# Jingliang-Duan/DSAC-v2

Measured on AMD Instinct MI355X. Metric: DSAC-T gradient steps/sec, batch=256 Humanoid (obs376/act17), higher is better.
Workload: dtype f32

## Files before the change

### dsac-v2_amd/csrc/dsact_api.hip

```cpp
#include <hip/hip_runtime.h>
#include <hip/hip_ext.h>
#include <dlfcn.h>
#include <chrono>
#include <stdarg.h>
#include <stdio.h>
#include <math.h>
#include <stdlib.h>
#include <string.h>

#include <algorithm>
#include <atomic>
#include <string>
#include <vector>

#include "../../include/dsact.h"
#include "dsact_kernels.h"
#include "dsact_chain.h"
#include "dsact_fat.h"
#include "dsact_act.h"
#include "dsact_act_batch.h"
#include "dsact_host_act.h"
#include "dsact_conv.h"

#define DSACT_KERNEL(group, ...) extern template __global__ void __VA_ARGS__;
// ... 2899 lines not shown
  if (cfg->conv_type != DSACT_CONV_NONE) {
    static const int k1[] = {8, 4, 3}, c1[] = {32, 64, 64}, s1[] = {4, 2, 1};
    static const int k2[] = {4, 3, 3, 3, 3, 3}, c2[] = {8, 16, 32, 64, 128, 256}, s2[] = {2, 2, 2, 2, 1, 1};
    if (cfg->conv_type != DSACT_CONV_TYPE_1 && cfg->conv_type != DSACT_CONV_TYPE_2) return fail(h, DSACT_E_INVALID, "conv_type must be 0, 1 (type_1) or 2 (type_2)");
    const bool t1 = cfg->conv_type == DSACT_CONV_TYPE_1;
    const int* ks = t1 ? k1 : k2; const int* cs = t1 ? c1 : c2; const int* ss = t1 ? s1 : s2;
    h->n_conv = t1 ? 3 : 6;
    if (cfg->img_c < 1 || cfg->img_h < 1 || cfg->img_w < 1 || (long long)cfg->img_c * cfg->img_h * cfg->img_w != cfg->obs_dim)
      return fail(h, DSACT_E_INVALID, "obs_dim must equal img_c*img_h*img_w for CNN nets");
    if (cfg->obs_dim % 4) return fail(h, DSACT_E_INVALID, "img_c*img_h*img_w must be a multiple of 4");
    int C = cfg->img_c, H = cfg->img_h, W = cfg->img_w;
    for (int j = 0; j < h->n_conv; ++j) {
      ConvGeom& g = h->cg[j];
      g.H = H; g.W = W; g.Cin = C; g.KS = ks[j]; g.stride = ss[j]; g.Cout = cs[j];
      g.OH = (H - g.KS) / g.stride + 1; g.OW = (W - g.KS) / g.stride + 1;
      if (H < g.KS || W < g.KS || g.OH < 1 || g.OW < 1) return fail(h, DSACT_E_INVALID, "image %dx%d too small for conv layer %d", cfg->img_h, cfg->img_w, j);
      g.K = g.KS * g.KS * g.Cin; g.KWC = g.KS * g.Cin; g.rowskip = g.W * g.Cin - g.KWC;
      g.inv_kwc = 1.0f / (float)g.KWC;
      if (g.KWC % 4) return fail(h, DSACT_E_INVALID, "kernel_width*channels of conv layer %d must be a multiple of 4 (got %d)", j, g.KWC);
      C = g.Cout; H = g.OH; W = g.OW;
    }
    h->cnn = true;
    h->cP = H * W;
    h->F = C * H * W;
    nblk = 2;
  }
  int pol_hidden[DSACT_MAX_HIDDEN_LAYERS] = {0};
  bool unequal = false;
  h->Lq = cfg->n_hidden;
  h->Lp = cfg->policy_n_hidden > 0 ? cfg->policy_n_hidden : cfg->n_hidden;
  if (h->Lp > DSACT_MAX_HIDDEN_LAYERS) return fail(h, DSACT_E_INVALID, "policy_n_hidden must be 0 (= n_hidden) or 1..%d", DSACT_MAX_HIDDEN_LAYERS);
  if (h->Lp != h->Lq && cfg->conv_type != DSACT_CONV_NONE) return fail(h, DSACT_E_INVALID, "policy_n_hidden: the CNN nets' MLP widths are fixed by conv_type");
  unequal = h->Lp != h->Lq;
  h->L = h->Lp > h->Lq ? h->Lp : h->Lq;
  for (int l = 0; l < h->Lp; ++l) {
    pol_hidden[l] = cfg->policy_hidden[l] > 0 ? cfg->policy_hidden[l] : (l < h->Lq ? cfg->hidden[l] : 0);
    if (pol_hidden[l] < 1 || pol_hidden[l] > kMaxWidth) return fail(h, DSACT_E_INVALID, "policy hidden width of layer %d must be 1..%d", l, kMaxWidth);
    unequal = unequal || l >= h->Lq || pol_hidden[l] != cfg->hidden[l];
  }
  if (unequal && (cfg->conv_type != DSACT_CONV_NONE || cfg->algo != 0))
    return fail(h, DSACT_E_INVALID, "value_hidden_sizes != policy_hidden_sizes is built for DSAC_V2 with MLP nets (tile-stage kernels)");
  const int nblk_pol = cfg->policy_twin ? 2 : nblk;
  h->unequal_widths = unequal || nblk_pol != nblk;
  for (int l = 0; l < h->L; ++l) {
    h->wq[l] = l < h->Lq ? nblk * cfg->hidden[l] : 0; h->wp[l] = l < h->Lp ? nblk_pol * pol_hidden[l] : 0;
    h->w[l] = h->wq[l] > h->wp[l] ? h->wq[l] : h->wp[l];
  }
  for (int l = 0; l < h->L; ++l)
    if (h->w[l] > kMaxWidth) return fail(h, DSACT_E_INVALID, "activation row width %d exceeds %d", h->w[l], kMaxWidth);
  h->ldx = (h->F + h->A + 3) & ~3;
  h->use_w1p = (size_t)4 * nblk * cfg->hidden[0] * h->ldx <= ((size_t)4 << 20);
  build_net(h->qd, h->F + h->A, cfg->hidden, h->Lq, 2, nblk, h->n_conv, h->cg);
  build_net(h->pd, h->F, pol_hidden, h->Lp, 2 * h->A, nblk_pol, h->n_conv, h->cg);
  h->n_q = h->qd.count; h->n_pi = h->pd.count;
  if (cfg->algo != DSACT_ALGO_DSAC_V2 && cfg->algo != DSACT_ALGO_DSAC_V1) return fail(h, DSACT_E_INVALID, "algo must be 0 (DSAC_V2) or 1 (DSAC_V1)");
  h->nq = cfg->algo == DSACT_ALGO_DSAC_V1 ? 1 : 2;
  h->n_online = h->nq * h->n_q + h->n_pi + 1;
  h->n_target = h->nq * h->n_q + h->n_pi;
  h->n_heads_wg = (h->B + 3) / 4;
  h->n_loss_wg = (h->B + 3) / 4;
  h->loss_rows = 4;
  h->auto_std_sums = h->B > 1024;
  if (const char* v = getenv("DSACT_TIMELINE_STAGE")) h->env_timeline_stage = v;
  { int v = 0; if (hipDeviceGetAttribute(&v, hipDeviceAttributeMultiprocessorCount, h->device) == hipSuccess && v > 0) h->n_cu = v; (void)hipGetLastError(); }
  h->env_no_pipe_defer = getenv("DSACT_NO_PIPE_DEFER") != nullptr;
  h->env_no_bqt = getenv("DSACT_NO_BQT_MERGE") != nullptr;
  h->env_no_bqp = getenv("DSACT_NO_BQP_MERGE") != nullptr;
  if (const char* v = getenv("DSACT_PIPE_MAP")) h->env_pipe_map = v;
  h->env_no_dcol_ident = getenv("DSACT_NO_DCOL_IDENT") != nullptr;
  h->env_no_fat_stage = getenv("DSACT_NO_FAT_STAGE") != nullptr;
  h->dw_chunks = (h->B > 448 && h->B % 256 == 0) ? h->B / 256 : 1;
  h->dw_part_stride = (h->n_online + 2 + 63) & ~(size_t)63;
  {
    const int R = 4 * h->cRG;
    bool ok = h->B % R == 0 && h->B % 16 == 0 && (h->B <= 256 || h->B % 256 == 0) &&
              getenv("DSACT_NO_CHAIN") == nullptr && !(h->nq == 1 && getenv("DSACT_NO_CHAIN_V1") != nullptr) &&
              !(h->cnn && (getenv("DSACT_NO_CHAIN_CNN") != nullptr || h->B > 1024));
    ok = ok && h->L <= kChMaxL;
    ok = ok && !h->unequal_widths;
    ok = ok && cfg->value_out_act != OUT_ACT_GELU && cfg->policy_out_act != OUT_ACT_GELU;
    for (int l = 0; l < h->L; ++l) ok = ok && cfg->hidden[l] == cfg->hidden[0];
    const int W0 = cfg->hidden[0];
    ok = ok && (W0 == 64 || W0 == 128 || W0 == 256);
    h->s_obs = roundup((h->F + 3) / 4, kPD);
    h->s_act = roundup((h->A + 3) / 4, kPD);
    h->SoT = roundup((2 * h->A + 3) / 4, kPD);
    ok = ok && (size_t)chain_lds(4 * (h->s_obs + h->s_act), W0, R).total * sizeof(float) <= 150 * 1024;
    h->chain_ok = ok;
    h->twin = ok && h->cnn;
    h->env_twin_seq = getenv("DSACT_TWIN_SEQ") != nullptr;
    if (ok) {
      const int per = (h->B > 1024 && h->B % 1024 == 0) ? 1024 : 256;
      h->dw_chunks = h->B > 1024 ? h->B / per : 1;
    }
    h->cW = W0; h->cNT = W0 / 64; h->n_slices = h->B / R;
    h->rg4_ok = ok && h->B % 16 == 0 &&
                (size_t)chain_lds(4 * (h->s_obs + h->s_act), W0, 16).total * sizeof(float) <= 150 * 1024;
    h->c_obs = (h->F + 15) / 16; h->c_act = (h->A + 15) / 16; h->c_out = (2 * h->A + 15) / 16;
    {
      const char* fm = getenv("DSACT_FAT_MIN");
      const int fat_min = fm ? atoi(fm) : 1024;
      h->fat = ok && !h->cnn && h->nq == 2 && h->B >= fat_min && h->B % 32 == 0 && (W0 == 128 || W0 == 256) &&
               cfg->value_out_act == 0 && cfg->policy_out_act == 0;
      h->fat_bwd = h->fat && h->B >= 4096;
      if (const char* v = getenv("DSACT_FAT_RT")) h->env_fat_rt = atoi(v) == 2 ? 2 : 1;
    }
    h->fwd_merge = ok && !h->cnn && h->B <= 256 && h->B / 4 <= kChainFlagSlices && chain_rg(h, 4) == 1 && getenv("DSACT_NO_FWD_MERGE") == nullptr;
    h->pi_merge = ok && !h->cnn && h->B <= 512 && !h->fat_bwd && getenv("DSACT_NO_PI_MERGE") == nullptr;
  }
  Carver c0;
  carve(h, c0, h->sets[0], SET_WS);
  h->ws_bytes = c0.off + 256;
  HIPCHK(h, hipMalloc(&h->ws, h->ws_bytes));
  HIPCHK(h, hipMemset(h->ws, 0, h->ws_bytes));
  Carver c1;
  c1.base = h->ws;
  carve(h, c1, h->sets[0], SET_WS);
  {
    DevState st0;
    memset(&st0, 0, sizeof(st0));
    st0.b1p_q = st0.b2p_q = st0.b1p_pi = st0.b2p_pi = st0.b1p_alpha = st0.b2p_alpha = 1.0;
    HIPCHK(h, hipMemcpy(h->st, &st0, sizeof(st0), hipMemcpyHostToDevice));
  }
  {
    std::vector<float> ones(h->B, 1.0f);
    HIPCHK(h, hipMemcpy(h->ones, ones.data(), h->B * sizeof(float), hipMemcpyHostToDevice));
  }
  if (h->cnn) {
    for (int j = 0; j < h->n_conv; ++j) {
      const ConvGeom& g = h->cg[j];
      if ((size_t)h->Brows * g.H * g.W * g.Cin > 2147483647ull || (size_t)h->Brows * g.OH * g.OW >= (1u << 24))
        return fail(h, DSACT_E_INVALID, "batch x image too large for the conv index arithmetic (layer %d)", j);
    }
    std::vector<int> iota(h->Brows);
    for (int i = 0; i < h->Brows; ++i) iota[i] = i;
    HIPCHK(h, hipMemcpy(h->idx_iota, iota.data(), iota.size() * sizeof(int), hipMemcpyHostToDevice));
  }
  HIPCHK(h, hipStreamCreateWithFlags(&h->stream, hipStreamNonBlocking));
  h->own_stream = true;
  for (const KernelFamily* f : kernels().all)
    for (int c = 0; c < f->n_cells; ++c)
      if (f->max_lds && f->cells[c]) HIPCHK(h, hipFuncSetAttribute(f->cells[c], hipFuncAttributeMaxDynamicSharedMemorySize, f->max_lds));
  HIPCHK(h, hipHostMalloc((void**)&h->handoff_host, 1024, hipHostMallocMapped));
  memset(h->handoff_host, 0, 1024);
  HIPCHK(h, hipHostGetDevicePointer((void**)&h->handoff_dev, h->handoff_host, 0));
  h->act_out_host = (unsigned long long*)(h->handoff_host + 32); h->act_out_dev = (unsigned long long*)(h->handoff_dev + 32);
  HIPCHK(h, hipMalloc((void**)&h->act_h, (size_t)kActMaxLayers * kMaxWidth * sizeof(unsigned long long)));
  HIPCHK(h, hipMemset(h->act_h, 0, (size_t)kActMaxLayers * kMaxWidth * sizeof(unsigned long long)));
  h->env_no_fast_act = getenv("DSACT_NO_FAST_ACT") != nullptr;
  h->host_act = getenv("DSACT_NO_HOST_ACT") == nullptr;

  if (h->fwd_merge) {
    int per_cu = 0;
    const size_t la = (size_t)chain_lds(4 * (h->s_obs + h->s_act), h->cW, 4 * chain_rg(h, 6)).total * sizeof(float);
    const void* fn = (const void*)kernels().chain_fwd2.find({h->cNT, false});
    if (!fn || hipOccupancyMaxActiveBlocksPerMultiprocessor(&per_cu, fn, 64 * h->cNT, la) != hipSuccess || per_cu < 2) h->fwd_merge = false;
    (void)hipGetLastError();
  }
  for (int i = 0; i < 8; ++i) {
    HIPCHK(h, hipHostMalloc((void**)&h->h_idx[i], (size_t)h->B * sizeof(int), hipHostMallocDefault));
    HIPCHK(h, hipEventCreateWithFlags(&h->h_idx_ev[i], hipEventDisableTiming));
  }
  return DSACT_OK;
}

int dsact_destroy(dsact_handle* h) {
  if (!h) return DSACT_E_INVALID;
  hipSetDevice(h->device);
  if (h->stream) hipStreamSynchronize(h->stream);
// ... 2390 lines not shown
```

### dsac-v2_amd/csrc/dsact_chain.h

```cpp
#pragma once
#include "dsact_kernels.h"

namespace dsact {

#ifndef DSACT_TILE_NAP
#define DSACT_TILE_NAP 24
#endif
constexpr int kChMaxL = 4;
#ifndef DSACT_KPD
#define DSACT_KPD 16
#endif
constexpr int kPD = DSACT_KPD;

#ifdef DSACT_TIMELINE
#define CTL(buf, k) do { if ((buf) && threadIdx.x == 0 && blockIdx.x < 1024) (buf)[blockIdx.x * 16 + (k)] = (long long)__builtin_readcyclecounter(); } while (0)
#define CTLR(buf, k) do { if ((buf) && threadIdx.x == 0 && blockIdx.x < 1024) (buf)[blockIdx.x * 16 + (k)] = (long long)__builtin_amdgcn_s_memrealtime(); } while (0)
#define CTLV(buf, k, v) do { if ((buf) && threadIdx.x == 0 && blockIdx.x < 1024) (buf)[blockIdx.x * 16 + (k)] = (long long)(v); } while (0)
#else
#define CTL(buf, k) do {} while (0)
#define CTLR(buf, k) do {} while (0)
#define CTLV(buf, k, v) do {} while (0)
#endif


struct WStr { f32x4 b[kPD]; };

__device__ __forceinline__ void stream_prologue(WStr& ws, const float* cur, int s_lo, int lane4) {
#pragma unroll
  for (int u = 0; u < kPD; ++u) ws.b[u] = gload4(cur + (size_t)(s_lo + u) * 256 + lane4);
}

__device__ __forceinline__ const float* uniform_ptr(const float* p) {
  const unsigned long long v = (unsigned long long)p;
  const unsigned lo = __builtin_amdgcn_readfirstlane((unsigned)v), hi = __builtin_amdgcn_readfirstlane((unsigned)(v >> 32));
  return (const float*)(((unsigned long long)hi << 32) | lo);
}
__device__ __forceinline__ const float* sgpr_ptr(const float* p) { p = uniform_ptr(p); asm("" : "+s"(p)); return p; }

template <int RG, bool TAIL = false>
__device__ __forceinline__ void gemm44_seg(WStr& ws, const float* cur, int s_lo, int s_hi, const float* nxt, int nxt_s0,
                                           bool has_nxt, const float* lds, int xs, int ld, int lane4, f32x4 (&acc)[RG][2],
                                           const float* tail = nullptr, int tail_c = 0, int tail_nt = 0) {
  static_assert(!TAIL || kPD >= 8, "the tail takes 8 slots of the stream");
  static_assert(kPD % 4 == 0, "one scalar base per 4 steps");
  constexpr bool SB = RG >= 2;
  f32x4 a0[RG], a1[RG];
#pragma unroll
  for (int g = 0; g < RG; ++g) a0[g] = *(const f32x4*)(lds + xs + 4 * g * ld + 4 * s_lo);
  for (int s0 = s_lo; s0 < s_hi; s0 += kPD) {
    const float* src = s0 + kPD < s_hi ? cur + (size_t)(s0 + kPD) * 256
                                       : (has_nxt ? nxt + (size_t)nxt_s0 * 256 : cur + (size_t)s_lo * 256);
    const bool at_tail = TAIL && tail != nullptr && !has_nxt && !(s0 + kPD < s_hi);
    const float* src8 = at_tail ? tail : src;
    const int tq = at_tail ? (tail_nt > 1 ? tail_c : 0) : 4;
    const float* sb[kPD / 4];
    if (SB) {
#pragma unroll
      for (int k = 0; k < kPD / 4; ++k) sb[k] = sgpr_ptr(TAIL && k < 2 ? src8 + (size_t)(k * tq) * 256 : src + (size_t)k * 1024);
    }
#pragma unroll
    for (int u = 0; u < kPD; ++u) {
      const int s = s0 + u;
#pragma unroll
      for (int g = 0; g < RG; ++g) {
        if (u & 1) a0[g] = *(const f32x4*)(lds + xs + 4 * g * ld + 4 * (s + 1));
        else a1[g] = *(const f32x4*)(lds + xs + 4 * g * ld + 4 * (s + 1));
      }
#pragma unroll
      for (int e = 0; e < 4; ++e) {
#pragma unroll
        for (int g = 0; g < RG; ++g)
          acc[g][e & 1] = __builtin_amdgcn_mfma_f32_4x4x1f32((u & 1) ? a1[g][e] : a0[g][e], ws.b[u][e], acc[g][e & 1], 0, 0, 0);
        if (e == 1) __builtin_amdgcn_sched_barrier(0);
      }
      if (SB) ws.b[u] = gload4(sb[u >> 2] + (size_t)(u & 3) * 256 + lane4);
      else if (TAIL && u < 8) ws.b[u] = gload4(src8 + (size_t)((u >> 2) * tq + (u & 3)) * 256 + lane4);
      else ws.b[u] = gload4(src + (size_t)u * 256 + lane4);
      __builtin_amdgcn_sched_barrier(0);
    }
  }
}

template <int NTO_MAX>
struct NarrowFrags { f32x4 w[NTO_MAX][4]; };

template <int NTO_MAX>
__device__ __forceinline__ void narrow_load(NarrowFrags<NTO_MAX>& f, const float* wf, int C, int nto, int wave, int lane4) {
#pragma unroll
  for (int t = 0; t < NTO_MAX; ++t) {
    if (t < nto) {
#pragma unroll
      for (int c = 0; c < 4; ++c) f.w[t][c] = gload4(wf + ((size_t)t * C + (size_t)wave * 4 + c) * 256 + lane4);
    }
  }
}
template <int NTO_MAX>
__device__ __forceinline__ void narrow_mma(const NarrowFrags<NTO_MAX>& f, int nto, int wave, float* lds, int xs, int red, int lane) {
  f32x4 a[4];
#pragma unroll
  for (int c = 0; c < 4; ++c) a[c] = *(const f32x4*)(lds + xs + 16 * (wave * 4 + c));
#pragma unroll
  for (int t = 0; t < NTO_MAX; ++t) {
    if (t < nto) {
      f32x4 acc = {0.f, 0.f, 0.f, 0.f};
#pragma unroll
      for (int c = 0; c < 4; ++c)
#pragma unroll
        for (int e = 0; e < 4; ++e) acc = __builtin_amdgcn_mfma_f32_16x16x4f32(f.w[t][c][e], a[c][e], acc, 0, 0, 0);
      *(f32x4*)(lds + red + ((wave * NTO_MAX + t) * 64 + lane) * 4) = acc;
    }
  }
}
template <int NTO_MAX, int NW>
__device__ __forceinline__ float narrow_get(const float* lds, int red, int m, int n) {
  const int t = n >> 4, ln = (((n & 15) >> 2) << 4) + m, e = n & 3;
  float s = lds[red + ((0 * NTO_MAX + t) * 64 + ln) * 4 + e];
#pragma unroll
  for (int w = 1; w < NW; ++w) s += lds[red + ((w * NTO_MAX + t) * 64 + ln) * 4 + e];
  return s;
}

template <int TPR>
__device__ __forceinline__ float rowN_sum(float v) {
  v += dpp_mov<0xB1>(v);
  v += dpp_mov<0x4E>(v);
  if (TPR >= 8) v += dpp_mov<0x141>(v);
  if (TPR >= 16) v += dpp_mov<0x140>(v);
  if (TPR >= 32) { float a, b; swap16(v, a, b); v = a + b; }
  if (TPR >= 64) { float a, b; swap32(v, a, b); v = a + b; }
  return v;
}

__device__ __forceinline__ bool chain_decode(int b, int n_units, int n_slices, int& unit, int& slice) {
  const int rep = n_units >= 5 ? 1 : (n_units >= 3 ? 2 : (n_units == 2 ? 4 : 8));
  const int xcd = b & 7, rnd = b >> 3;
  if (xcd >= n_units * rep) return false;
  unit = xcd % n_units;
  slice = rnd * rep + xcd / n_units;
  return slice < n_slices;
}
inline int chain_grid(int n_units, int n_slices) {
  const int rep = n_units >= 5 ? 1 : (n_units >= 3 ? 2 : (n_units == 2 ? 4 : 8));
  return 8 * ((n_slices + rep - 1) / rep);
}
struct XcdMap { int unit[8], base[8], stride[8]; };
inline XcdMap xcd_map_uniform(int n_units) {
  XcdMap m;
  const int rep = n_units >= 5 ? 1 : (n_units >= 3 ? 2 : (n_units == 2 ? 4 : 8));
  for (int x = 0; x < 8; ++x) {
    const bool on = x < n_units * rep;
    m.unit[x] = on ? x % n_units : -1; m.base[x] = on ? x / n_units : 0; m.stride[x] = rep;
  }
  return m;
}
inline XcdMap xcd_map_shares(int n_units, const int* share) {
  XcdMap m;
  int x = 0;
  for (int u = 0; u < n_units; ++u)
    for (int k = 0; k < share[u] && x < 8; ++k, ++x) { m.unit[x] = u; m.base[x] = k; m.stride[x] = share[u]; }
  for (; x < 8; ++x) { m.unit[x] = -1; m.base[x] = 0; m.stride[x] = 1; }
  return m;
// ... 413 lines not shown
      const int a0 = f0 ? __hip_atomic_load(f0, __ATOMIC_RELAXED, __HIP_MEMORY_SCOPE_AGENT) : 1;
      const int a1 = f1 ? __hip_atomic_load(f1, __ATOMIC_RELAXED, __HIP_MEMORY_SCOPE_AGENT) : 1;
      if (a0 && a1) break;
      if (++spins > (1 << 17)) { if (timeout) *timeout = 1; break; }
      __builtin_amdgcn_s_sleep(16);
    }
  }
  __syncthreads();
}

constexpr int kArriveStride = 64;
__device__ __forceinline__ void pack_store4(float* p, const f32x4& v, int agent) {
  if (agent) asm volatile("global_store_dwordx4 %0, %1, off sc1" : : "v"(p), "v"(v) : "memory");
  else nt_store4(p, v);
}
__device__ __forceinline__ void hand_store(float* p, float v, int agent) {
  if (agent) st_agent(p, v); else *p = v;
}
__device__ __forceinline__ void chain_arrive(int* cnt) {
  if (!cnt) return;
  stores_acked_barrier();
  if (threadIdx.x < 8) __hip_atomic_fetch_add(cnt + threadIdx.x * kArriveStride, 1, __ATOMIC_RELAXED, __HIP_MEMORY_SCOPE_AGENT);
}
struct ArriveWait {
  const int* cnt; int need; int* timeout;
  long long* tl = nullptr;
  int quick = 0;
  int kind = 0;
  __device__ __forceinline__ void operator()() const {
    if (threadIdx.x == 0) {
      const int* c = cnt + ((int)blockIdx.x & 7) * kArriveStride;
      int spins = 0;
      while (__hip_atomic_load(c, __ATOMIC_RELAXED, __HIP_MEMORY_SCOPE_AGENT) < need) {
        if (++spins > (1 << 17)) { if (timeout) *timeout = 1; break; }
        if (quick) __builtin_amdgcn_s_sleep(4); else __builtin_amdgcn_s_sleep(DSACT_TILE_NAP);
      }
    }
    asm volatile("s_barrier" ::: "memory");
    CTLR(tl, 13);
  }
  __device__ __forceinline__ void stamp_class(int v) const { CTLV(tl, 11, kind | v); }
};

__device__ __forceinline__ bool fwd_decode(const FwdArgs& a, int b, int& unit, int& slice) {
  const int x = b & 7;
  unit = a.map.unit[x];
  if (unit < 0) return false;
  slice = a.map.base[x] + a.map.stride[x] * (b >> 3);
  return slice < a.u[unit].n_slices;
}
inline int fwd_grid(const FwdArgs& a) {
  int rounds = 0;
  for (int x = 0; x < 8; ++x) {
    if (a.map.unit[x] < 0) continue;
    const int n = a.u[a.map.unit[x]].n_slices - a.map.base[x];
    const int r = n > 0 ? (n + a.map.stride[x] - 1) / a.map.stride[x] : 0;
    rounds = r > rounds ? r : rounds;
  }
  return 8 * rounds;
}

template <int NW, int RG, bool GA = false, typename AT = FwdArgs, typename UT = FwdUnit>
__device__ __forceinline__ void chain_fwd_body(const AT& a, const UT& u, int unit, int slice, float* lds) {
  constexpr int W = 64 * NW, SH = W / 4, R = 4 * RG, NTHR = 64 * NW, TPR = NTHR / R;
  int* const done_flag = (u.done && !(a.debug_withhold && unit == 0 && slice == 0)) ? u.done + slice : nullptr;
  const int tid = threadIdx.x, lane = tid & 63;
  const int wave = __builtin_amdgcn_readfirstlane(tid >> 6);
  const int lane4 = lane * 4;
  const int n = 64 * wave + lane;
  const int row0 = slice * R;
  const int L = a.L, F = a.F, A = a.A;
  const int S0 = a.s_obs + u.s_act;
  const int head = u.head & HEAD_KIND, twin = u.head & (HEAD_TWIN_FIRST | HEAD_TWIN_SECOND);
  const int c_out = ((u.head >> 8) & 0xff) ? ((u.head >> 8) & 0xff) : W / 16;
  const int oact = GA ? head_out_act(u.head) : 0;
  const ChainLds S = chain_lds(4 * (a.s_obs + a.s_act), W, R);
  const int xin = S.off_in, red = S.off_red;
  CTL(a.timeline, 0);
  CTLR(a.timeline, 14);
  const bool do_obs = u.seg != SEG_ACT_FROM_SAVED;
  const bool do_act = u.seg != SEG_OBS_ONLY && u.s_act > 0;
  WStr ws;
  const float* w0 = u.wf[0] + (size_t)wave * (S0 + a.tpad) * 256;
  stream_prologue(ws, w0, do_obs ? 0 : a.s_obs, lane4);
  float bq[kChMaxL];
#pragma unroll
  for (int l = 0; l < kChMaxL; ++l) bq[l] = u.bias[l < L ? l : 0][n];
  const int mr = tid / TPR, jr = tid % TPR;
  constexpr int NQ = (32 + TPR - 1) / TPR;
  float pre_eps[NQ], pre_bmu[NQ], pre_braw[NQ], pre_s[NQ], pre_c[NQ];
#pragma unroll
  for (int q = 0; q < NQ; ++q) { pre_eps[q] = 0.f; pre_bmu[q] = 0.f; pre_braw[q] = 0.f; pre_s[q] = 1.f; pre_c[q] = 0.f; }
  if (head == HEAD_POLICY) {
#pragma unroll
    for (int q = 0; q < NQ; ++q) {
      const int d = jr + q * TPR;
      if (d < A) {
        pre_eps[q] = u.eps[(size_t)(row0 + mr) * A + d];
        pre_bmu[q] = u.bias[L][d]; pre_braw[q] = u.bias[L][A + d];
        pre_s[q] = a.act_scale[d]; pre_c[q] = a.act_center[d];
      }
    }
  } else if (head == HEAD_Q && jr == 0) {
    pre_bmu[0] = u.bias[L][0]; pre_braw[0] = u.bias[L][1];
  }
  const bool pairs_in = (u.late_wait & HW_PAIRS_IN) != 0, pairs_out = (u.late_wait & HW_PAIRS_OUT) != 0;
  const unsigned tag = (pairs_in || pairs_out) ? (unsigned)(*a.tagp) + 1u : 0u;
  const bool head_wait = (u.late_wait & HW_HEAD) != 0;
  const int* const flag0 = (pairs_in || head_wait) ? nullptr : u.wait0;
  const bool waits = flag0 || u.wait1 || pairs_in;
  const bool late = waits && (u.late_wait & HW_LATE) && u.seg != SEG_ACT_FROM_SAVED && u.s_act > 0;
  if ((flag0 || u.wait1) && !late)
    chain_wait(flag0 ? flag0 + row0 / u.wait_rows0 : nullptr, u.wait1 ? u.wait1 + row0 / u.wait_rows1 : nullptr, a.spin_timeout);
  f32x4 zi[RG];
  if (u.seg == SEG_ACT_FROM_SAVED) {
#pragma unroll
    for (int g = 0; g < RG; ++g)
#pragma unroll
      for (int r = 0; r < 4; ++r) zi[g][r] = ld_agent(u.zinit + (size_t)(row0 + 4 * g + r) * W + n);
  }
  auto stage_act = [&]() {
    const int Fp = 4 * a.s_obs;
    if (pairs_in) {
      const unsigned long long* hp = (const unsigned long long*)u.wait0;
      const int per_row = 4 * u.s_act;
      for (int e = tid; e < R * per_row; e += NTHR) {
        const int r = e / per_row, k = e % per_row;
        float v = 0.0f;
        if (k < A) {
          const unsigned long long* src = hp + (size_t)(row0 + r) * 32 + k;
          unsigned long long pv = __hip_atomic_load(src, __ATOMIC_RELAXED, __HIP_MEMORY_SCOPE_AGENT);
          int spins = 0;
          while ((unsigned)(pv >> 32) != tag) {
            if (++spins > (1 << 17)) { if (a.spin_timeout) *a.spin_timeout = 1; break; }
            __builtin_amdgcn_s_sleep(8);
            pv = __hip_atomic_load(src, __ATOMIC_RELAXED, __HIP_MEMORY_SCOPE_AGENT);
          }
          v = __builtin_bit_cast(float, (unsigned)pv);
        }
        lds[xin + r * S.ld_in + Fp + k] = v;
      }
      return;
    }
    const int aq = u.s_act, total = R * aq;
    for (int e = tid; e < total; e += NTHR) {
      const int r = e / aq, k = (e % aq) * 4;
      f32x4 v = {0.f, 0.f, 0.f, 0.f};
      const float* s = u.x + (size_t)(row0 + r) * a.ldx + F + k;
      for (int c = 0; c < 4; ++c) if (k + c < A) v[c] = ld_agent(s + c);
      *(f32x4*)(lds + xin + r * S.ld_in + Fp + k) = v;
    }
  };
  {
    const int Fp = 4 * a.s_obs;
    if (do_obs) {
      const int fq = Fp >> 2, total = R * fq;
      for (int e0 = tid; e0 < total; e0 += 4 * NTHR) {
        f32x4 v[4];
#pragma unroll
        for (int q = 0; q < 4; ++q) {
          const int e = e0 + q * NTHR;
          const int r = e < total ? e / fq : 0, k = e < total ? (e % fq) * 4 : 0;
          const float* s = u.x + (size_t)(row0 + r) * a.ldx + (k + 3 < F ? k : 0);
          v[q] = *(const f32x4u*)s;
        }
#pragma unroll
        for (int q = 0; q < 4; ++q) {
          const int e = e0 + q * NTHR;
          if (e < total) {
            const int r = e / fq, k = (e % fq) * 4;
            f32x4 o = v[q];
            if (k + 3 >= F) {
              const float* s = u.x + (size_t)(row0 + r) * a.ldx;
              for (int c = 0; c < 4; ++c) o[c] = k + c < F ? s[k + c] : 0.0f;
            }
            *(f32x4*)(lds + xin + r * S.ld_in + k) = o;
          }
        }
      }
    }
    if (do_act && !late) stage_act();
  }
  f32x4 acc[RG][2];
#pragma unroll
  for (int g = 0; g < RG; ++g) { acc[g][0] = f32x4{0.f, 0.f, 0.f, 0.f}; acc[g][1] = acc[g][0]; }
  if (u.seg == SEG_ACT_FROM_SAVED) {
#pragma unroll
    for (int g = 0; g < RG; ++g) acc[g][0] = zi[g];
  }
  lds_barrier();
  CTL(a.timeline, 1);
  if (u.x0t) {
    const int K0 = F + (do_act ? A : 0);
    for (int e = tid; e < K0 * RG; e += NTHR) {
      const int k = e / RG, g4 = e % RG;
      const int kk = k < F ? k : 4 * a.s_obs + (k - F);
      f32x4 v;
#pragma unroll
      for (int r = 0; r < 4; ++r) v[r] = lds[xin + (4 * g4 + r) * S.ld_in + kk];
      nt_store4(u.x0t + pk_index(k, row0 + 4 * g4, a.Cb), v);
    }
  }
  const int xs_in = xin + (lane & 3) * S.ld_in;
  const bool more = L > 1;
  const float* w1 = u.wf[more ? 1 : 0] + (size_t)wave * (more ? SH + a.tpad : S0 + a.tpad) * 256;
  if (do_obs) {
    const bool into_act = do_act;
    gemm44_seg<RG>(ws, w0, 0, a.s_obs, into_act ? w0 : w1, into_act ? a.s_obs : 0, into_act || (more && u.seg != SEG_OBS_ONLY),
                   lds, xs_in, S.ld_in, lane4, acc);
    if (u.zsave) {
#pragma unroll
      for (int g = 0; g < RG; ++g) {
        const f32x4 v = acc[g][0] + acc[g][1];
#pragma unroll
        for (int r = 0; r < 4; ++r) st_agent(u.zsave + (size_t)(row0 + 4 * g + r) * W + n, v[r]);
      }
      if (u.zdone) chain_publish(u.zdone + slice);
    }
    CTL(a.timeline, 2);
    if (u.seg == SEG_OBS_ONLY) { CTLR(a.timeline, 15); chain_publish(done_flag); return; }
    if (u.seg == SEG_FULL_SPLIT) {
#pragma unroll
      for (int g = 0; g < RG; ++g) { acc[g][0] = acc[g][0] + acc[g][1]; acc[g][1] = f32x4{0.f, 0.f, 0.f, 0.f}; }
    }
  }
  if (late) {
    if (flag0 || u.wait1)
      chain_wait(flag0 ? flag0 + row0 / u.wait_rows0 : nullptr, u.wait1 ? u.wait1 + row0 / u.wait_rows1 : nullptr, a.spin_timeout);
    stage_act();
    lds_barrier();
  }
  if (do_act) gemm44_seg<RG>(ws, w0, a.s_obs, S0, w1, 0, more, lds, xs_in, S.ld_in, lane4, acc);
  CTL(a.timeline, 3);
  NarrowFrags<4> hf;
  const int nto = head == HEAD_POLICY ? (2 * A + 15) >> 4 : 1;
  for (int l = 0; l < L; ++l) {
    if (l == L - 1 && head != HEAD_NONE) narrow_load<4>(hf, u.wf[L], c_out, nto, wave, lane4);
    const int hn = (l & 1) ? S.off_h1 : S.off_h0;
    const float bl = l == 0 ? bq[0] : l == 1 ? bq[1] : l == 2 ? bq[2] : bq[3];
#pragma unroll
    for (int g = 0; g < RG; ++g) {
      const f32x4 z = acc[g][0] + acc[g][1] + bl;
      f32x4 hv, gd;
      if (GA) act4(u.act, z, hv, gd); else gelu4(z, hv, gd);
#pragma unroll
      for (int r = 0; r < 4; ++r) lds[hn + (4 * g + r) * S.ld_h + n] = hv[r];
      if (u.H[l]) nt_store4(u.H[l] + pk_index(n, row0 + 4 * g, a.Cb), hv);
      if (u.G[l]) nt_store4(u.G[l] + pk_index(n, row0 + 4 * g, a.Cb), gd);
      acc[g][0] = f32x4{0.f, 0.f, 0.f, 0.f}; acc[g][1] = acc[g][0];
    }
    lds_barrier();
    CTL(a.timeline, 4 + 2 * l);
    if (l + 1 < L) {
      const float* wc = u.wf[l + 1] + (size_t)wave * (SH + a.tpad) * 256;
      const bool has_nxt = l + 2 < L;
      const float* wn = u.wf[has_nxt ? l + 2 : l + 1] + (size_t)wave * (SH + a.tpad) * 256;
      gemm44_seg<RG>(ws, wc, 0, SH, wn, 0, has_nxt, lds, hn + (lane & 3) * S.ld_h, S.ld_h, lane4, acc);
      CTL(a.timeline, 5 + 2 * l);
    }
  }
  if (head == HEAD_NONE) { CTLR(a.timeline, 15); chain_publish(done_flag); return; }
  const int hl = ((L - 1) & 1) ? S.off_h1 : S.off_h0;
  narrow_mma<4>(hf, nto, wave, lds, hl + ((lane & 15) & (R - 1)) * S.ld_h + 4 * (lane >> 4), red, lane);
  lds_barrier();
  CTL(a.timeline, 12);
  float* const carry = lds + S.off_carry;
  if (twin == HEAD_TWIN_FIRST) {
    for (int e = tid; e < R * 16 * nto; e += NTHR) {
      const int mm = e / (16 * nto), o = e % (16 * nto);
      const float v = narrow_get<4, NW>(lds, red, mm, o);
      if (u.qout) st_agent(u.qout + (size_t)(row0 + mm) * 64 + o, v);
      else carry[mm * 64 + o] = v;
    }
    CTLR(a.timeline, 15);
    if (u.qout) chain_publish(done_flag);
    return;
  }
  const bool add_carry = twin == HEAD_TWIN_SECOND;
  if (head_wait) {
    chain_wait(u.wait0 + row0 / u.wait_rows0, nullptr, a.spin_timeout);
    for (int e = tid; e < R * 16 * nto; e += NTHR) {
      const int mm = e / (16 * nto), o = e % (16 * nto);
      carry[mm * 64 + o] = ld_agent(u.zinit + (size_t)(row0 + mm) * 64 + o);
    }
    lds_barrier();
  }
  const int m = mr, j = jr;
  const int r = row0 + m;
  if (head == HEAD_Q) {
    if (j == 0) {
      float mean = narrow_get<4, NW>(lds, red, m, 0), raw = narrow_get<4, NW>(lds, red, m, 1);
      if (add_carry) { mean += carry[m * 64]; raw += carry[m * 64 + 1]; }
      mean += pre_bmu[0]; raw += pre_braw[0];
      float sgm = 1.0f;
      if (GA && oact) { mean = out_act_fwd(oact, mean); raw = out_act_fwd(oact, raw); sgm = out_act_grad_y(oact, raw); }
      u.qout[2 * r] = mean; u.qout[2 * r + 1] = raw;
      if (u.qstd) { u.qstd[2 * r] = softplus(raw); u.qstd[2 * r + 1] = softplus_grad(raw) * sgm; }
    }
    CTL(a.timeline, 13);
    CTLR(a.timeline, 15);
    chain_publish(done_flag);
    return;
  }
  float lp = 0.f, s_tanh = 0.f, s_sig = 0.f;
#pragma unroll
  for (int q = 0; q < NQ; ++q) {
    const int d = j + q * TPR;
    if (d >= A) break;
    float mu = narrow_get<4, NW>(lds, red, m, d), raw = narrow_get<4, NW>(lds, red, m, A + d);
    if (add_carry) { mu += carry[m * 64 + d]; raw += carry[m * 64 + A + d]; }
    mu += pre_bmu[q]; raw += pre_braw[q];
    if (GA && oact) { mu = out_act_fwd(oact, mu); if (!(u.head & HEAD_STD_PLAIN)) raw = out_act_fwd(oact, raw); }
    const TanhGaussFwd f = tanh_gauss_fwd(mu, raw, pre_eps[q], pre_s[q], pre_c[q], a.lo_ls, a.hi_ls);
    lp += f.lp;
    st_agent(u.xact + (size_t)r * a.ldx + F + d, f.a);
// ... 359 lines not shown
    } else narrow_load<2>(af, u.w1at, c1at, nta, wave, lane4);
  }
  narrow_mma<2>(af, nta, wave, lds, (cur ? S.off_h1 : S.off_h0) + ((lane & 15) & (R - 1)) * S.ld_h + 4 * (lane >> 4), red, lane);
  lds_barrier();
  const unsigned ptag = (MRG && u.dA_pairs) ? (unsigned)(*a.tagp) + 1u : 0u;
  for (int d = j; d < 16 * nta; d += TPR) {
    const float v = d < a.A ? narrow_get<2, NW>(lds, red, m, d) : 0.0f;
    u.dA[(size_t)r * 32 + d] = v;
    if (MRG && u.dA_pairs)
      __hip_atomic_store(u.dA_pairs + (size_t)r * 32 + d, ((unsigned long long)ptag << 32) | (unsigned long long)__builtin_bit_cast(unsigned, v),
                         __ATOMIC_RELAXED, __HIP_MEMORY_SCOPE_AGENT);
  }
  CTL(a.timeline, 12);
  CTLR(a.timeline, 15);
}

template <int NW, int RG>
__global__ void __launch_bounds__(256) k_chain_bwd_q(BwdQArgs a) {
  extern __shared__ __attribute__((aligned(16))) float lds[];
  if ((int)blockIdx.x >= a.n_chain_blocks) { loss_rider(a.ride); return; }
  bwd_q_body<NW, RG>(a, (int)blockIdx.x, lds);
}

struct BwdPiArgs {
  int n_trunks;
  const float* woutT1; const float* wb1[kChMaxL]; const float* G1[kChMaxL]; float* dZ1[kChMaxL];
  const float* dA2[2];
  float* dz0row; int ldz0;
  const float* dA[2];
  const float* logits_pi; const float* eps_new; const float* log_alpha;
  const float* woutT; int SoT;
  const float* wb[kChMaxL];
  const float* G[kChMaxL];
  float* dZ[kChMaxL];
  float* dout_pi; float* d_new_act;
  float* dout_piT;
  int n_slices, B, A, L, Cb;
  float inv_B; int auto_alpha; float alpha_fixed;
  int pi_out_act, pi_out_n;
  const float* act_scale; float lo_ls, hi_ls;
  const float* part_loss; int n_part; float target_entropy; float* grad_log_alpha;
  int n_chain_blocks;
  int tile0, n_extra;
  int merge_dw, pi_tile0, n_pi_tiles, finalize;
  int* cnt_pi; int* spin_timeout;
  const unsigned long long* dA_pairs[2]; const long long* tagp;
  int debug_withhold;
  long long* timeline;
  Dw2Args dw;
};

__device__ __forceinline__ void bwd_pi_alpha_grad(const BwdPiArgs& a, int lane) {
  float s = 0.f;
  for (int r0 = 0; r0 < a.n_part; r0 += 64) {
    const int rr = r0 + lane;
    s += rr < a.n_part ? a.part_loss[(size_t)rr * kLossPart + 7] : 0.f;
  }
  s = wave_sum(s);
  if (lane == 0) a.grad_log_alpha[0] = a.auto_alpha ? -(s * a.inv_B + a.target_entropy) : 0.0f;
}

template <int NW, int RG>
__device__ __forceinline__ void bwd_pi_body(const BwdPiArgs& a, int slice, float* lds, int trunk = 0) {
  constexpr int W = 64 * NW, SH = W / 4, R = 4 * RG, NTHR = 64 * NW, TPR = NTHR / R;
  const int tid = threadIdx.x;
  if (slice >= a.n_slices || tid >= NTHR) return;
  const bool lead = trunk == 0;
  const float* const* const t_wb = trunk ? a.wb1 : a.wb;
  const float* const* const t_G = trunk ? a.G1 : a.G;
  float* const* const t_dZ = trunk ? a.dZ1 : a.dZ;
  float* const dz0row = a.dz0row ? a.dz0row + trunk * W : nullptr;
  const int lane = tid & 63;
  const int wave = __builtin_amdgcn_readfirstlane(tid >> 6);
  const int lane4 = lane * 4;
  const int n = 64 * wave + lane;
  const int row0 = slice * R;
  const int L = a.L, A = a.A;
  const ChainLds S = chain_lds(4 * a.SoT, W, R);
  float* xdo = lds + S.off_in;
  CTL(a.timeline, 0);
  CTLR(a.timeline, 14);
  WStr ws;
  const float* wo = (trunk ? a.woutT1 : a.woutT) + (size_t)wave * a.SoT * 256;
  stream_prologue(ws, wo, 0, lane4);
  const int m = tid / TPR, j = tid % TPR;
  const int r = row0 + m;
  constexpr int NQ = (32 + TPR - 1) / TPR;
  float pdA[NQ], pmu[NQ], praw[NQ], peps[NQ], psc[NQ];
  const bool pairs = a.dA_pairs[0] != nullptr;
#pragma unroll
  for (int q = 0; q < NQ; ++q) {
    const int d = j + q * TPR;
    const bool ok = d < A;
    pdA[q] = (ok && !pairs) ? a.dA[0][(size_t)r * 32 + d] + a.dA[1][(size_t)r * 32 + d] : 0.f;
    if (a.dA2[0] && ok) pdA[q] += a.dA2[0][(size_t)r * 32 + d] + a.dA2[1][(size_t)r * 32 + d];
    pmu[q] = ok ? a.logits_pi[(size_t)r * 2 * A + d] : 0.f;
    praw[q] = ok ? a.logits_pi[(size_t)r * 2 * A + A + d] : 0.f;
    peps[q] = ok ? a.eps_new[(size_t)r * A + d] : 0.f;
    psc[q] = ok ? a.act_scale[d] : 1.f;
  }
  if (pairs) {
    const unsigned tag = (unsigned)(*a.tagp) + 1u;
#pragma unroll
    for (int q = 0; q < NQ; ++q) {
      const int d = j + q * TPR;
      if (d < A) {
        float v[2];
#pragma unroll
        for (int c = 0; c < 2; ++c) {
          const unsigned long long* src = a.dA_pairs[c] + (size_t)r * 32 + d;
          unsigned long long pv = __hip_atomic_load(src, __ATOMIC_RELAXED, __HIP_MEMORY_SCOPE_AGENT);
          int spins = 0;
          while ((unsigned)(pv >> 32) != tag) {
            if (++spins > (1 << 17)) { if (a.spin_timeout) *a.spin_timeout = 1; break; }
            __builtin_amdgcn_s_sleep(8);
            pv = __hip_atomic_load(src, __ATOMIC_RELAXED, __HIP_MEMORY_SCOPE_AGENT);
          }
          v[c] = __builtin_bit_cast(float, (unsigned)pv);
        }
        pdA[q] = v[0] + v[1];
      }
    }
  }
  if (slice == 0 && wave == 0 && !a.merge_dw && lead) bwd_pi_alpha_grad(a, lane);
  const int agent = a.merge_dw;
  const float alpha = a.auto_alpha ? expf(a.log_alpha[0]) : a.alpha_fixed;
  for (int e = tid; e < R * 4 * a.SoT; e += NTHR) xdo[(e / (4 * a.SoT)) * S.ld_in + e % (4 * a.SoT)] = 0.0f;
  lds_barrier();
#pragma unroll
  for (int q = 0; q < NQ; ++q) {
    const int d = j + q * TPR;
    if (d >= A) break;
    const float dA = pdA[q];
    float dmu, draw;
    tanh_gauss_bwd(pmu[q], praw[q], peps[q], psc[q], a.lo_ls, a.hi_ls, dA, alpha * a.inv_B, dmu, draw);
    if (a.pi_out_act) {
      dmu *= out_act_grad_y(a.pi_out_act, pmu[q]);
      if (A + d < a.pi_out_n) draw *= out_act_grad_y(a.pi_out_act, praw[q]);
    }
    if (lead) {
      a.dout_pi[(size_t)r * 2 * A + d] = dmu;
      a.dout_pi[(size_t)r * 2 * A + A + d] = draw;
      hand_store(a.dout_piT + pk_index(d, r, a.Cb), dmu, agent);
      hand_store(a.dout_piT + pk_index(A + d, r, a.Cb), draw, agent);
      a.d_new_act[(size_t)r * A + d] = dA;
    }
    xdo[m * S.ld_in + d] = dmu;
    xdo[m * S.ld_in + A + d] = draw;
  }
  lds_barrier();
  CTL(a.timeline, 1);
  f32x4 acc[RG][2];
  {
#pragma unroll
    for (int g = 0; g < RG; ++g) { acc[g][0] = f32x4{0.f, 0.f, 0.f, 0.f}; acc[g][1] = acc[g][0]; }
    f32x4 gq[RG];
#pragma unroll
    for (int g = 0; g < RG; ++g) gq[g] = gload4(t_G[L - 1] + pk_index(n, row0 + 4 * g, a.Cb));
    const bool has_nxt = L > 1;
    gemm44_seg<RG>(ws, wo, 0, a.SoT, has_nxt ? t_wb[L - 1] + (size_t)wave * SH * 256 : wo, 0, has_nxt,
                   lds, S.off_in + (lane & 3) * S.ld_in, S.ld_in, lane4, acc);
#pragma unroll
    for (int g = 0; g < RG; ++g) {
      const f32x4 dz = (acc[g][0] + acc[g][1]) * gq[g];
#pragma unroll
      for (int rr = 0; rr < 4; ++rr) lds[S.off_h0 + (4 * g + rr) * S.ld_h + n] = dz[rr];
      pack_store4(t_dZ[L - 1] + pk_index(n, row0 + 4 * g, a.Cb), dz, agent);
    }
    lds_barrier();
    if (dz0row && L == 1) store_dz0_rows<W, R, NTHR>(dz0row, a.ldz0, row0, lds + S.off_h0, S.ld_h);
    CTL(a.timeline, 2);
  }
  int cur = 0;
  for (int l = L - 1; l >= 1; --l) {
#pragma unroll
    for (int g = 0; g < RG; ++g) { acc[g][0] = f32x4{0.f, 0.f, 0.f, 0.f}; acc[g][1] = acc[g][0]; }
    f32x4 gq[RG];
#pragma unroll
    for (int g = 0; g < RG; ++g) gq[g] = gload4(t_G[l - 1] + pk_index(n, row0 + 4 * g, a.Cb));
    const bool has_nxt = l > 1;
    gemm44_seg<RG>(ws, t_wb[l] + (size_t)wave * SH * 256, 0, SH, t_wb[has_nxt ? l - 1 : l] + (size_t)wave * SH * 256, 0, has_nxt,
                   lds, (cur ? S.off_h1 : S.off_h0) + (lane & 3) * S.ld_h, S.ld_h, lane4, acc);
    const int hn = cur ? S.off_h0 : S.off_h1;
#pragma unroll
    for (int g = 0; g < RG; ++g) {
      const f32x4 dz = (acc[g][0] + acc[g][1]) * gq[g];
#pragma unroll
      for (int rr = 0; rr < 4; ++rr) lds[hn + (4 * g + rr) * S.ld_h + n] = dz[rr];
      pack_store4(t_dZ[l - 1] + pk_index(n, row0 + 4 * g, a.Cb), dz, agent);
    }
    cur ^= 1;
    if (l > 1 || dz0row) lds_barrier();
    if (dz0row && l == 1) store_dz0_rows<W, R, NTHR>(dz0row, a.ldz0, row0, lds + hn, S.ld_h);
    CTL(a.timeline, 3 + (L - 1 - l));
  }
  CTLR(a.timeline, 15);
  if (a.merge_dw && !(a.debug_withhold && slice == 0)) chain_arrive(a.cnt_pi);
}

__device__ __forceinline__ const int* pi_tile_counter(const BwdPiArgs& a, int) { return a.cnt_pi; }

__device__ __forceinline__ void bwd_pi_tail_blocks(const BwdPiArgs& a, int idx, float* lds) {
  const int per_range = xcd_chunk_grid(a.n_extra);
  const int n_rider_blocks = a.merge_dw ? per_range : 0x7fffffff;
  int t;
  if (idx < n_rider_blocks) {
    if (!xcd_chunk(idx % per_range, a.n_extra, t)) return;
    CTLR(a.timeline, 14);
    dw2_tile(a.dw, (idx / per_range) * a.dw.n_base + a.tile0 + t, lds);
    CTLR(a.timeline, 15);
    return;
  }
  idx -= n_rider_blocks;
  if (idx < xcd_chunk_grid(a.n_pi_tiles)) {
    if (!xcd_chunk(idx, a.n_pi_tiles, t)) return;
    dw2_tile<2, ArriveWait>(a.dw, a.pi_tile0 + t, lds, ArriveWait{pi_tile_counter(a, a.pi_tile0 + t), a.n_slices, a.spin_timeout});
    return;
  }
  ArriveWait{a.cnt_pi, a.n_slices, a.spin_timeout}();
  if (threadIdx.x < 64) {
    bwd_pi_alpha_grad(a, (int)threadIdx.x);
    if (a.finalize && threadIdx.x == 0) finalize_update(a.dw.fo);
  }
}

template <int NW, int RG>
__global__ void __launch_bounds__(256) k_chain_bwd_pi(BwdPiArgs a) {
  extern __shared__ __attribute__((aligned(16))) float lds[];
  if ((int)blockIdx.x >= a.n_chain_blocks) { bwd_pi_tail_blocks(a, (int)blockIdx.x - a.n_chain_blocks, lds); return; }
  const int per = a.n_chain_blocks >> 1, b = (int)blockIdx.x;
  const int trunk = (a.n_trunks == 2 && b >= per) ? 1 : 0;
  bwd_pi_body<NW, RG>(a, trunk ? b - per : b, lds, trunk);
}

struct BwdQtArgs {
  BwdQArgsN<4> q;
  Dw2Args dw;
  const int* tile_tab; int n_tile_blocks;
  int n_riders;
  int need;
  int* spin_timeout;
  const float* logp_new; int n_part; float target_entropy; float* grad_log_alpha; int finalize;
};
static_assert(sizeof(BwdQtArgs) <= 4096, "kernel arguments are limited to 4 KB");
// ... 141 lines not shown
```

Baseline: 18780.

## Pad chain input segments to 4-step granule and run short MFMA trips

Input segment step counts (obs, act, output-transpose) are now rounded up to a multiple of 4 rather than to the full 16-slot stream depth. A new gemm44_short streams weights in quads and handles a partial last trip of 4, 8 or 12 steps, and the prefetch redirects to the next segment or layer when the current one runs out. This removes the MFMA and weight-load work spent on zero padding, which is large for obs=376 and act=17. In exchange the stream-source selection logic becomes more complex, with more branches per quad and a risk of weight-layout mismatch wherever the padding is assumed elsewhere.

Result: no change. 18810 (median of 4 runs) (+0.1%).

```diff
diff --git a/dsac-v2_amd/csrc/dsact_api.hip b/dsac-v2_amd/csrc/dsact_api.hip
--- a/dsac-v2_amd/csrc/dsact_api.hip
+++ b/dsac-v2_amd/csrc/dsact_api.hip
@@ -3005,9 +3005,9 @@
     for (int l = 0; l < h->L; ++l) ok = ok && cfg->hidden[l] == cfg->hidden[0];
     const int W0 = cfg->hidden[0];
     ok = ok && (W0 == 64 || W0 == 128 || W0 == 256);
-    h->s_obs = roundup((h->F + 3) / 4, kPD);
-    h->s_act = roundup((h->A + 3) / 4, kPD);
-    h->SoT = roundup((2 * h->A + 3) / 4, kPD);
+    h->s_obs = seg_steps(h->F);
+    h->s_act = seg_steps(h->A);
+    h->SoT = seg_steps(2 * h->A);
     ok = ok && (size_t)chain_lds(4 * (h->s_obs + h->s_act), W0, R).total * sizeof(float) <= 150 * 1024;
     h->chain_ok = ok;
     h->twin = ok && h->cnn;
diff --git a/dsac-v2_amd/csrc/dsact_chain.h b/dsac-v2_amd/csrc/dsact_chain.h
--- a/dsac-v2_amd/csrc/dsact_chain.h
+++ b/dsac-v2_amd/csrc/dsact_chain.h
@@ -11,6 +11,12 @@
 #define DSACT_KPD 16
 #endif
 constexpr int kPD = DSACT_KPD;
+#ifndef DSACT_SEG_GRANULE
+#define DSACT_SEG_GRANULE 4
+#endif
+constexpr int kSegG = DSACT_SEG_GRANULE;
+static_assert(kSegG == 4 || kSegG == kPD, "a quad of slots has one source; kPD: whole trips everywhere, as before the short trips");
+__host__ __device__ inline int seg_steps(int K) { return ((K + 3) / 4 + kSegG - 1) / kSegG * kSegG; }
 
 #ifdef DSACT_TIMELINE
 #define CTL(buf, k) do { if ((buf) && threadIdx.x == 0 && blockIdx.x < 1024) (buf)[blockIdx.x * 16 + (k)] = (long long)__builtin_readcyclecounter(); } while (0)
@@ -30,6 +36,26 @@
   for (int u = 0; u < kPD; ++u) ws.b[u] = gload4(cur + (size_t)(s_lo + u) * 256 + lane4);
 }
 
+struct StreamNext {
+  const float* nxt; int n_nxt;
+  const float* nxt2;
+  bool has_nxt, has_nxt2;
+};
+__device__ __forceinline__ const float* stream_quad(const float* cur, int n, int j, int q, const StreamNext& N) {
+  if (j < n) return cur + (size_t)j * 256;
+  if (N.has_nxt && 4 * q < N.n_nxt) return N.nxt + (size_t)(4 * q) * 256;
+  if (N.has_nxt && N.has_nxt2) return N.nxt2 + (size_t)(4 * q) * 256;
+  return cur;
+}
+__device__ __forceinline__ void stream_prologue_short(WStr& ws, const float* cur, int n, const StreamNext& N, int lane4) {
+#pragma unroll
+  for (int q = 0; q < kPD / 4; ++q) {
+    const float* b = stream_quad(cur, n, 4 * q, q, N);
+#pragma unroll
+    for (int i = 0; i < 4; ++i) ws.b[4 * q + i] = gload4(b + (size_t)i * 256 + lane4);
+  }
+}
+
 __device__ __forceinline__ const float* uniform_ptr(const float* p) {
   const unsigned long long v = (unsigned long long)p;
   const unsigned lo = __builtin_amdgcn_readfirstlane((unsigned)v), hi = __builtin_amdgcn_readfirstlane((unsigned)(v >> 32));
@@ -77,6 +103,61 @@
       else if (TAIL && u < 8) ws.b[u] = gload4(src8 + (size_t)((u >> 2) * tq + (u & 3)) * 256 + lane4);
       else ws.b[u] = gload4(src + (size_t)u * 256 + lane4);
       __builtin_amdgcn_sched_barrier(0);
+    }
+  }
+}
+
+template <int RG, int Q>
+__device__ __forceinline__ void gemm44_quad(WStr& ws, const float* sb, int j0, const float* lds, int xs, int ld, int lane4,
+                                            f32x4 (&a0)[RG], f32x4 (&a1)[RG], f32x4 (&acc)[RG][2]) {
+#pragma unroll
+  for (int i = 0; i < 4; ++i) {
+    constexpr int u0 = 4 * Q;
+    const int u = u0 + i, s = j0 + u;
+#pragma unroll
+    for (int g = 0; g < RG; ++g) {
+      if (u & 1) a0[g] = *(const f32x4*)(lds + xs + 4 * g * ld + 4 * (s + 1));
+      else a1[g] = *(const f32x4*)(lds + xs + 4 * g * ld + 4 * (s + 1));
+    }
+#pragma unroll
+    for (int e = 0; e < 4; ++e) {
+#pragma unroll
+      for (int g = 0; g < RG; ++g)
+        acc[g][e & 1] = __builtin_amdgcn_mfma_f32_4x4x1f32((u & 1) ? a1[g][e] : a0[g][e], ws.b[u][e], acc[g][e & 1], 0, 0, 0);
+      if (e == 1) __builtin_amdgcn_sched_barrier(0);
+    }
+    ws.b[u] = gload4(sb + (size_t)i * 256 + lane4);
+    __builtin_amdgcn_sched_barrier(0);
+  }
+}
+
+template <int RG>
+__device__ __forceinline__ void gemm44_short(WStr& ws, const float* cur, int n, const StreamNext& N, const float* lds, int xs,
+                                             int ld, int lane4, f32x4 (&acc)[RG][2]) {
+  static_assert(kPD == 16, "four quads per trip");
+  constexpr bool SB = RG >= 2;
+  f32x4 a0[RG], a1[RG];
+#pragma unroll
+  for (int g = 0; g < RG; ++g) a0[g] = *(const f32x4*)(lds + xs + 4 * g * ld);
+  int j0 = 0;
+  for (; j0 + kPD <= n; j0 += kPD) {
+    const float* sb[4];
+#pragma unroll
+    for (int q = 0; q < 4; ++q) { const float* p = stream_quad(cur, n, j0 + kPD + 4 * q, q, N); sb[q] = SB ? sgpr_ptr(p) : uniform_ptr(p); }
+    gemm44_quad<RG, 0>(ws, sb[0], j0, lds, xs, ld, lane4, a0, a1, acc);
+    gemm44_quad<RG, 1>(ws, sb[1], j0, lds, xs, ld, lane4, a0, a1, acc);
+    gemm44_quad<RG, 2>(ws, sb[2], j0, lds, xs, ld, lane4, a0, a1, acc);
+    gemm44_quad<RG, 3>(ws, sb[3], j0, lds, xs, ld, lane4, a0, a1, acc);
+  }
+  const int m = n - j0;
+  if (m > 0) {
+    const float* sb[3];
+#pragma unroll
+    for (int q = 0; q < 3; ++q) { const float* p = stream_quad(cur, n, n, q, N); sb[q] = SB ? sgpr_ptr(p) : uniform_ptr(p); }
+    gemm44_quad<RG, 0>(ws, sb[0], j0, lds, xs, ld, lane4, a0, a1, acc);
+    if (m > 4) {
+      gemm44_quad<RG, 1>(ws, sb[1], j0, lds, xs, ld, lane4, a0, a1, acc);
+      if (m > 8) gemm44_quad<RG, 2>(ws, sb[2], j0, lds, xs, ld, lane4, a0, a1, acc);
     }
   }
 }
@@ -656,7 +737,15 @@
   const bool do_act = u.seg != SEG_OBS_ONLY && u.s_act > 0;
   WStr ws;
   const float* w0 = u.wf[0] + (size_t)wave * (S0 + a.tpad) * 256;
-  stream_prologue(ws, w0, do_obs ? 0 : a.s_obs, lane4);
+  {
+    const bool more0 = L > 1;
+    const float* w1p = u.wf[more0 ? 1 : 0] + (size_t)wave * (more0 ? SH + a.tpad : S0 + a.tpad) * 256;
+    const StreamNext nx_act0 = {w1p, SH, w1p, more0, false};
+    const StreamNext nx_obs0 = do_act ? StreamNext{w0 + (size_t)a.s_obs * 256, u.s_act, w1p, true, more0}
+                                      : StreamNext{w1p, SH, w1p, more0 && u.seg != SEG_OBS_ONLY, false};
+    if (do_obs) stream_prologue_short(ws, w0, a.s_obs, nx_obs0, lane4);
+    else stream_prologue_short(ws, w0 + (size_t)a.s_obs * 256, u.s_act, nx_act0, lane4);
+  }
   float bq[kChMaxL];
 #pragma unroll
   for (int l = 0; l < kChMaxL; ++l) bq[l] = u.bias[l < L ? l : 0][n];
@@ -760,7 +849,7 @@
   for (int g = 0; g < RG; ++g) { acc[g][0] = f32x4{0.f, 0.f, 0.f, 0.f}; acc[g][1] = acc[g][0]; }
   if (u.seg == SEG_ACT_FROM_SAVED) {
 #pragma unroll
-    for (int g = 0; g < RG; ++g) acc[g][0] = zi[g];
+    for (int g = 0; g < RG; ++g) { acc[g][0] = zi[g]; asm volatile("" : "+v"(acc[g][0])); }
   }
   lds_barrier();
   CTL(a.timeline, 1);
@@ -778,10 +867,13 @@
   const int xs_in = xin + (lane & 3) * S.ld_in;
   const bool more = L > 1;
   const float* w1 = u.wf[more ? 1 : 0] + (size_t)wave * (more ? SH + a.tpad : S0 + a.tpad) * 256;
+  const float* const wact = w0 + (size_t)a.s_obs * 256;
+  const StreamNext nx_act = {w1, SH, w1, more, false};
   if (do_obs) {
     const bool into_act = do_act;
-    gemm44_seg<RG>(ws, w0, 0, a.s_obs, into_act ? w0 : w1, into_act ? a.s_obs : 0, into_act || (more && u.seg != SEG_OBS_ONLY),
-                   lds, xs_in, S.ld_in, lane4, acc);
+    const StreamNext nx_obs = into_act ? StreamNext{wact, u.s_act, w1, true, more}
+                                       : StreamNext{w1, SH, w1, more && u.seg != SEG_OBS_ONLY, false};
+    gemm44_short<RG>(ws, w0, a.s_obs, nx_obs, lds, xs_in, S.ld_in, lane4, acc);
     if (u.zsave) {
 #pragma unroll
       for (int g = 0; g < RG; ++g) {
@@ -804,7 +896,7 @@
     stage_act();
     lds_barrier();
   }
-  if (do_act) gemm44_seg<RG>(ws, w0, a.s_obs, S0, w1, 0, more, lds, xs_in, S.ld_in, lane4, acc);
+  if (do_act) gemm44_short<RG>(ws, wact, u.s_act, nx_act, lds, xs_in + 4 * a.s_obs, S.ld_in, lane4, acc);
   CTL(a.timeline, 3);
   NarrowFrags<4> hf;
   const int nto = head == HEAD_POLICY ? (2 * A + 15) >> 4 : 1;
@@ -1330,7 +1422,8 @@
   CTLR(a.timeline, 14);
   WStr ws;
   const float* wo = (trunk ? a.woutT1 : a.woutT) + (size_t)wave * a.SoT * 256;
-  stream_prologue(ws, wo, 0, lane4);
+  const StreamNext nx_out = {L > 1 ? t_wb[L - 1] + (size_t)wave * SH * 256 : wo, SH, wo, L > 1, false};
+  stream_prologue_short(ws, wo, a.SoT, nx_out, lane4);
   const int m = tid / TPR, j = tid % TPR;
   const int r = row0 + m;
   constexpr int NQ = (32 + TPR - 1) / TPR;
@@ -1405,9 +1498,7 @@
     f32x4 gq[RG];
 #pragma unroll
     for (int g = 0; g < RG; ++g) gq[g] = gload4(t_G[L - 1] + pk_index(n, row0 + 4 * g, a.Cb));
-    const bool has_nxt = L > 1;
-    gemm44_seg<RG>(ws, wo, 0, a.SoT, has_nxt ? t_wb[L - 1] + (size_t)wave * SH * 256 : wo, 0, has_nxt,
-                   lds, S.off_in + (lane & 3) * S.ld_in, S.ld_in, lane4, acc);
+    gemm44_short<RG>(ws, wo, a.SoT, nx_out, lds, S.off_in + (lane & 3) * S.ld_in, S.ld_in, lane4, acc);
 #pragma unroll
     for (int g = 0; g < RG; ++g) {
       const f32x4 dz = (acc[g][0] + acc[g][1]) * gq[g];
```
